# CloudEngineHub/dexrobot_isaac

Measured on AMD Instinct MI355X. Metric: env-steps/sec BlindGrasping num_envs=4096 per MI355X (random actions), higher is better.
Workload: dtype f32

## Files before the change

### dexrobot_isaac_amd/build.py

```python
import os
import shutil
import subprocess

HERE = os.path.dirname(os.path.abspath(__file__))
CSRC = os.path.join(HERE, "csrc")
LIB = os.path.join(HERE, "libdexsim.so")
SOURCES = ["dexsim.hip", "dexsim_device.h", "dexsim_physics.hip.inc", "dexsim_l2.hip.inc"]


DEBUG_SPIN_LIB = os.path.join(HERE, "libdexsim_dbgspin.so")


def _stale(lib=LIB):
    if not os.path.exists(lib):
        return True
    t = os.path.getmtime(lib)
    deps = [os.path.join(CSRC, s) for s in SOURCES] + [os.path.join(HERE, "..", "include", "dexsim.h")]
    return any(os.path.getmtime(d) > t for d in deps if os.path.exists(d))


def build_debug_spin(force=False, bound=2000000):
    return build_lib(force=force, defs=(f"-DDEXSIM_DEBUG_SPIN={int(bound)}",), out=DEBUG_SPIN_LIB)


def build_lib(force=False, verbose=False, defs=(), out=None):
    lib = out or LIB
    if not force and not _stale(lib):
        return lib
    hipcc = shutil.which("hipcc") or "/opt/rocm/bin/hipcc"
    if not os.path.exists(hipcc):
        raise RuntimeError("hipcc not found: libdexsim.so cannot be built on this machine")
    cmd = [hipcc, "--offload-arch=gfx950", "-O3", "-fno-slp-vectorize", "-fno-hip-fp32-correctly-rounded-divide-sqrt",
           "-mllvm", "-amdgpu-sched-strategy=max-ilp", "-fPIC", "-shared", "-std=c++17", *defs,
           "-o", lib, os.path.join(CSRC, "dexsim.hip")]
    if verbose:
        print(" ".join(cmd))
    subprocess.check_call(cmd, cwd=CSRC)
    return lib


if __name__ == "__main__":
    print(build_lib(force=True, verbose=True))
```

### dexrobot_isaac_amd/csrc/dexsim_device.h

```cpp
#pragma once
#include <hip/hip_runtime.h>

#include "../../include/dexsim.h"

#define DEXSIM_FIELDS(X)                                                                                    \
                                \
  X(float, q, 26) X(float, qd, 26) X(float, targets, 26)                                                    \
  X(float, box_pos, 3) X(float, box_quat, 4) X(float, box_lin, 3) X(float, box_ang, 3)                      \
  X(float, box_mass, 1) X(float, box_mu, 1)                                                                 \
                                                \
  X(float, site_pose, 77) X(float, hand_vel, 6) X(float, cforce, 51) X(float, cf5, 15)                      \
                                                    \
  X(float, jframe, 156) X(float, ufree, 32) X(float, fac_finv, 60)                                          \
  X(float, fac_g, 120) X(int, ncontact, 1) X(float, cgeom, DEXSIM_KMAX * 8) X(int, ccode, DEXSIM_KMAX)      \
  X(float, crow, DEXSIM_KMAX * 3 * 28) X(float, crowq, DEXSIM_KMAX * 3 * 28 + 4) X(float, clam, DEXSIM_KMAX * 3) X(float, chdr, DEXSIM_KMAX * 8) X(float, cstage, 6 * NP_STAGE * 9)                                         \
   \
  X(float, wlam, DEXSIM_NWKEY * 4) X(int, wgen, 1) X(int, csplit, 1)                                         \
        \
  X(float, active_prev_targets, 18) X(float, active_rule_targets, 18) X(float, prev_actions, 18)            \
  X(float, actions, 18) X(float, prev_dof_pos, 26)                                                          \
  X(float, contact_duration_steps, 5) X(float, prev_contact_binary, 5) X(int, episode_step, 1)              \
  X(int, success_duration_steps, 1) X(int, success_conditions_met, 1) X(int, current_stage, 1)              \
  X(int, just2, 1) X(int, just3, 1) X(float, time_in_stage, 1) X(float, stage_contact_duration, 1)          \
  X(float, initial_box_pos, 3)                                                                              \
// ... 33 lines not shown
  float box_inv_I_k;
  float base_A[4][3], base_Oc[4][3], base_Q3z[4];
  unsigned obs_div_magic;
  int inertia_diag;
  float hand_reach;
  int obs_col_row[DEXSIM_OBS_ALL_DIM];
  JC jc[DEXSIM_NJ];
  Arena arena;
};

#define CNT_ANY_RESET 0
#define CNT_SUCC 1
#define CNT_FAIL 2
#define CNT_TERM_SUCCESS 8
#define CNT_TERM_FAILURE 9
#define CNT_TERM_TIMEOUT 10
#define CNT_NUM_RESETS 11
#define CNT_CONTACTS 16
#define CNT_HAND_CONTACTS 18
#define CNT_SPIN_TIMEOUT 20
#define CNT_PHYS_STEPS 13
#define CNT_CONSECUTIVE 14
#define CNT_RC_FIRST 15

typedef float f2 __attribute__((ext_vector_type(2)));
typedef float f4 __attribute__((ext_vector_type(4)));
__device__ __forceinline__ void st4_global(float* p, f4 v) { *(__attribute__((address_space(1))) f4*)p = v; }
__device__ __forceinline__ void st4_global(float* p, float a, float b, float c, float d) { f4 v; v.x = a; v.y = b; v.z = c; v.w = d; st4_global(p, v); }

struct V3 { float x, y, z; };
struct Q4 { float x, y, z, w; };
struct S6 { float xx, yy, zz, xy, xz, yz; };
struct M3 { float m[9]; };

#define DI __device__ __forceinline__

DI V3 v3(float x, float y, float z) { return {x, y, z}; }
DI V3 v3p(const float* p) { return {p[0], p[1], p[2]}; }
DI V3 operator+(V3 a, V3 b) { return {a.x + b.x, a.y + b.y, a.z + b.z}; }
DI V3 operator-(V3 a, V3 b) { return {a.x - b.x, a.y - b.y, a.z - b.z}; }
DI V3 operator*(float s, V3 a) { return {s * a.x, s * a.y, s * a.z}; }
DI V3& operator+=(V3& a, V3 b) { a.x += b.x; a.y += b.y; a.z += b.z; return a; }
DI V3& operator-=(V3& a, V3 b) { a.x -= b.x; a.y -= b.y; a.z -= b.z; return a; }
DI float dot(V3 a, V3 b) { return a.x * b.x + a.y * b.y + a.z * b.z; }
DI V3 cross(V3 a, V3 b) { return {a.y * b.z - a.z * b.y, a.z * b.x - a.x * b.z, a.x * b.y - a.y * b.x}; }
DI float norm(V3 a) { return sqrtf(dot(a, a)); }
// ... 171 lines not shown
```

### dexrobot_isaac_amd/csrc/dexsim_l2.hip.inc

```

struct CouplingGroup { int n, dof[3]; float scale[3]; };
constexpr CouplingGroup kCoupling[18] = {
    {1, {0}, {1}}, {1, {1}, {1}}, {1, {2}, {1}}, {1, {3}, {1}}, {1, {4}, {1}}, {1, {5}, {1}},
    {1, {6}, {1}},
    {1, {7}, {1}},
    {2, {8, 9}, {1, 1}},
    {3, {10, 18, 22}, {1, 1, 2}},
    {1, {11}, {1}}, {2, {12, 13}, {1, 1}},
    {1, {15}, {1}}, {2, {16, 17}, {1, 1}},
    {1, {19}, {1}}, {2, {20, 21}, {1, 1}},
    {1, {23}, {1}}, {2, {24, 25}, {1, 1}},
};
constexpr int kHeldDof = 14;
constexpr int kActiveFingerDof[12] = {8, 7, 6, 10, 12, 11, 16, 15, 20, 19, 24, 23};

enum {
#define X(name, dim) O_##name, O_##name##_last = O_##name + (dim) - 1,
  DEXSIM_OBS_KEYS(X)
#undef X
  O_end
};
static_assert(O_end == DEXSIM_OBS_ALL_DIM, "DEXSIM_OBS_ALL_DIM is not the sum of the DEXSIM_OBS_KEYS dims");
static_assert(O_object_pos == DEXSIM_OBS_BASE_TASK_DIM, "DEXSIM_OBS_BASE_TASK_DIM is not the row of object_pos");

DI void begin_step_counters(int* cnt, int stamp) {
  const int o = (stamp & 1) ^ 1;
  cnt[CNT_CONTACTS + o] = 0; cnt[CNT_HAND_CONTACTS + o] = 0;
}

DI void actions_block(const Arena& A, const ApiPtrs& T, const DevParams* __restrict__ P, const float* __restrict__ act,
                      int zero_targets, int N, int NR) {
  const int wv = threadIdx.x >> 6, lane = threadIdx.x & 63;
  const int e = blockIdx.x * 64 + lane;
  const DexSimConfig& C = P->cfg;
  const int na = C.num_actions;
  const bool real = e < NR;
  if (blockIdx.x == 0 && threadIdx.x == 0) begin_step_counters(T.counters, T.stamp);
  const int fs = C.policy_controls_base ? 6 : 0;
  if (wv == 0) {
    FLD(targets, kHeldDof) = 0.f;
    if (real && T.full_dof_targets) T.full_dof_targets[(size_t)e * 26 + kHeldDof] = 0.f;
  }
#pragma unroll
  for (int i = 0; i < 18; i++) {
    if (i / 3 != wv) continue;
    const float ai = (real && i < na) ? act[(size_t)e * na + i] : 0.f;
    const int ci = i < 6 ? i : fs + (i - 6);
    const bool driven = i < 6 ? (C.policy_controls_base != 0) : (C.policy_controls_fingers != 0);
    const float ac = (driven && real && ci < na) ? act[(size_t)e * na + ci] : 0.f;
    float raw = FLD(active_rule_targets, i);
    const float prev = FLD(active_prev_targets, i);
    FLD(actions, i) = ai;
    if (T.actions_copy && real && i < na) T.actions_copy[(size_t)e * na + i] = ai;
    if (T.raw_targets && !zero_targets) {
      raw = real ? T.raw_targets[(size_t)e * 18 + i] : raw;
    } else if (C.control_mode == DEXSIM_MODE_POSITION_DELTA) {
      if (driven) raw = prev + ac * C.max_deltas[i];
      raw = clampf(raw, C.active_lower[i], C.active_upper[i]);
    } else {
      if (driven) raw = (ac + 1.0f) * 0.5f * (C.active_upper[i] - C.active_lower[i]) + C.active_lower[i];
    }
    const float d = clampf(raw - prev, -C.max_deltas[i], C.max_deltas[i]);
    const float nxt = clampf(prev + d, C.active_lower[i], C.active_upper[i]);
    if (!zero_targets) FLD(active_prev_targets, i) = nxt;
    const float tgt = zero_targets ? 0.f : nxt;
    const CouplingGroup& g = kCoupling[i];
#define PUT(k) do { const float t = tgt * g.scale[k]; FLD(targets, g.dof[k]) = t; \
                    if (real && T.full_dof_targets) T.full_dof_targets[(size_t)e * 26 + g.dof[k]] = t; } while (0)
    PUT(0);
    if (g.n > 1) PUT(1);
    if (g.n > 2) PUT(2);
#undef PUT
    FLD(prev_actions, i) = ai;
  }
}

__global__ __launch_bounds__(384) void k_actions(Arena A, ApiPtrs T, const DevParams* __restrict__ P, const float* __restrict__ act,
                                                 int zero_targets, int N, int NR) {
  actions_block(P->arena, T, P, act, zero_targets, N, NR);
}

DI V3 site_pos(const Arena& A, int N, int e, int s) { return {FLD(site_pose, 7 * s), FLD(site_pose, 7 * s + 1), FLD(site_pose, 7 * s + 2)}; }
DI Q4 site_quat(const Arena& A, int N, int e, int s) {
  return {FLD(site_pose, 7 * s + 3), FLD(site_pose, 7 * s + 4), FLD(site_pose, 7 * s + 5), FLD(site_pose, 7 * s + 6)};
}
#define OB_STRIDE (DEXSIM_OBS_ALL_DIM + 1)
#define OB(i) s_ob[lane * OB_STRIDE + (i)]

#ifdef DEXSIM_PROFILE_PHASES
#define PB_STAMP(k) do { if (threadIdx.x == 0) A.crow[(size_t)(32 + (k)) * N + blockIdx.x * 64] = __int_as_float((int)(__builtin_amdgcn_s_memtime() - pb_t0)); } while (0)
#else
#define PB_STAMP(k) do {} while (0)
#endif
#define ST_PEN 0
#define ST_FV2 1
#define ST_FA2 2
#define ST_RC 3
#define ST_WORDS (ST_RC + DEXSIM_NUM_REWROWS + 1)
#define ST(i) s_st[(i) * 64 + lane]
#define POST_NTASK 12

DI void post_task(int t, const Arena& A, const DevParams* __restrict__ P, const int* __restrict__ cnt, float* s_ob, float* s_st,
// ... 540 lines not shown
    for (int g = wv; g < (DEXSIM_NUM_REWROWS + 1 + 3) / 4; g += nw) {
      const int row = 4 * g + r4;
      if (row <= DEXSIM_NUM_REWROWS) {
        const float* sr = s_st + (ST_RC + row) * 64 + 4 * l16;
        const f4 v = {sr[0], sr[1], sr[2], sr[3]};
        float* dst = row < DEXSIM_NUM_REWROWS ? A.rew_comp + (size_t)row * N : A.rew;
        st4_global(dst + blockIdx.x * 64 + 4 * l16, v);
      }
    }
  }
  POST_STAMP();
  POST_STAMP();
#undef POST_STAMP
}

#define POST_LDS_BYTES ((64 * OB_STRIDE + 64 * ST_WORDS + DEXSIM_OBS_ALL_DIM) * sizeof(float))
__global__ __launch_bounds__(512) void k_post(Arena A, ApiPtrs T, const DevParams* __restrict__ P, int* __restrict__ cnt,
                                              int obs_only, int fold_reset, int N, int NR) {
  extern __shared__ float s_post[];
  post_block(P->arena, T, P, cnt, s_post, obs_only, fold_reset, N, NR, 0);
}

DI void finalize_stats(const ApiPtrs& T, const DevParams* __restrict__ P, int NR) {
  int* cnt = T.counters;
  float* st = T.stats;
  const DexSimConfig& C = P->cfg;
  auto mean = [&](int count) { return (float)((double)count / (double)NR); };
  st[DEXSIM_STAT_SUCC_MEAN] = mean(cnt[CNT_SUCC]);
  for (int i = 0; i < DEXSIM_NUM_FAIL; i++) st[DEXSIM_STAT_FAIL_MEAN + i] = mean(cnt[CNT_FAIL + i]);
  st[DEXSIM_STAT_SUCCESS_RATE] = mean(cnt[CNT_TERM_SUCCESS]);
  st[DEXSIM_STAT_FAILURE_RATE] = mean(cnt[CNT_TERM_FAILURE]);
  st[DEXSIM_STAT_TIMEOUT_RATE] = mean(cnt[CNT_TERM_TIMEOUT]);
  int cs = cnt[CNT_TERM_SUCCESS] > 0 ? cnt[CNT_CONSECUTIVE] + 1 : 0;
  if (cs > C.max_consecutive_successes) cs = C.max_consecutive_successes;
  cnt[CNT_CONSECUTIVE] = cs;
  st[DEXSIM_STAT_CONSECUTIVE_SUCCESSES] = (float)cs;
  st[DEXSIM_STAT_NUM_RESETS] = (float)cnt[CNT_NUM_RESETS];
  st[DEXSIM_STAT_PHYSICS_STEPS] = cnt[CNT_ANY_RESET] == T.stamp ? 2.f : 1.f;
  st[DEXSIM_STAT_MEAN_CONTACTS] = mean(cnt[CNT_CONTACTS + (T.stamp & 1)]);
  st[DEXSIM_STAT_MEAN_HAND_CONTACTS] = mean(cnt[CNT_HAND_CONTACTS + (T.stamp & 1)]);
  cnt[CNT_RC_FIRST] = 0;
  for (int i = CNT_SUCC; i <= CNT_NUM_RESETS; i++) cnt[i] = 0;
  if (T.sink_stats)
    for (int i = 0; i < DEXSIM_STAT_USED; i++) T.sink_stats[i] = st[i];
}

DI void reset_phase1(const Arena& A, int N, int e) {
#pragma unroll
  for (int f = 0; f < 5; f++) { FLD(contact_duration_steps, f) = 0.f; FLD(prev_contact_binary, f) = 0.f; }
#pragma unroll
  for (int i = 0; i < 26; i++) FLD(prev_dof_pos, i) = 0.f;
#pragma unroll
  for (int i = 0; i < 18; i++) FLD(prev_actions, i) = 0.f;
}

DI void reset_phase0(const Arena& A, const ApiPtrs& T, const DevParams* __restrict__ P, int N, int NR, int e) {
  const DexSimConfig& C = P->cfg;
  FLD(episode_success, 0) = 0; FLD(episode_failure, 0) = 0; FLD(success_reason, 0) = 0;
#pragma unroll
  for (int i = 0; i < DEXSIM_NUM_FAIL; i++) FLD(failure_reason, i) = 0;
  FLD(episode_step, 0) = 0;
  T.episode_step_count[e] = 0;
  T.episode_length[e] = 0;
  if (T.masks) {
#pragma unroll
    for (int i = 0; i < DEXSIM_NUM_SUCC + DEXSIM_NUM_FAIL; i++) T.masks[(size_t)(DEXSIM_MASK_SUCC_REASON + i) * NR + e] = 0;
  }
// ... 41 lines not shown
  }
#pragma unroll
  for (int c = 0; c < 18; c++) {
    const CouplingGroup& g = kCoupling[c];
    FLD(active_prev_targets, c) = q[g.dof[g.n - 1]] / g.scale[g.n - 1];
  }
}

__global__ __launch_bounds__(64) void k_reset(Arena A, ApiPtrs T, const DevParams* __restrict__ P, const int64_t* __restrict__ ids, int k,
                                              int mode, int phase, int N, int NR) {
  int e = blockIdx.x * 64 + threadIdx.x;
  if (mode == 3) {
    if (e >= NR || FLD(reset_flag, 0) == 0) return;
  } else {
    if (e >= k) return;
    if (mode == 1) e = (int)ids[e];
    if (e < 0 || e >= NR) return;
  }
  if (phase == 1) reset_phase1(A, N, e);
  else reset_phase0(A, T, P, N, NR, e);
}

__global__ void k_finalize(ApiPtrs T, const DevParams* __restrict__ P, int NR) {
  if (threadIdx.x != 0 || blockIdx.x != 0) return;
  finalize_stats(T, P, NR);
}

__global__ void k_begin_step(int* cnt, int stamp) {
  if (threadIdx.x == 0 && blockIdx.x == 0) begin_step_counters(cnt, stamp);
}

__global__ __launch_bounds__(64) void k_init(Arena A, ApiPtrs T, const DevParams* __restrict__ P, int N, int NR) {
  const int e = blockIdx.x * 64 + threadIdx.x;
  const DexSimConfig& C = P->cfg;
  FLD(box_quat, 3) = 1.f;
  FLD(box_pos, 2) = C.box_z;
  FLD(initial_box_pos, 2) = C.box_z;
  if (C.box_fixed) {
#pragma unroll
    for (int i = 0; i < 3; i++) { FLD(box_pos, i) = C.box_fixed_pos[i]; FLD(initial_box_pos, i) = C.box_fixed_pos[i]; }
  }
  float mass = C.box_mass > 0.f ? C.box_mass : 1.f, mu = C.box_friction;
  if (C.dr_enabled) {
    uint32_t x[4];
    philox4x32(x, (uint32_t)e, 0u, 0u, 0u, C.dr_seed, 0xd12au);
    mass = C.dr_mass_lo + u01(x[0]) * (C.dr_mass_hi - C.dr_mass_lo);
    mu = C.dr_mu_lo + u01(x[1]) * (C.dr_mu_hi - C.dr_mu_lo);
// ... 24 lines not shown
```

### dexrobot_isaac_amd/csrc/dexsim_physics.hip.inc

```

#define GPTR(p) ((__attribute__((address_space(1))) __typeof__(*(p))*)(p))
#define FLD(f, r) GPTR(A.f)[(size_t)(r) * N + e]
#define ROWADDR(w, lane) ((((w) >> 2) * 64 + (lane)) * 4 + ((w) & 3))

DI int wave_role(int w) { return w == 2 ? 5 : ((w >= 3 && w <= 5) ? w - 1 : w); }
#ifndef SPEC_SPLIT_NUM
#define SPEC_SPLIT_NUM 12
#endif

#define CODE_TYPE(c) ((c) & 3)
#define CODE_CAP(c) (((c) >> 2) & 31)
#define CODE_SAMPLE(c) (((c) >> 7) & 7)
#define CODE_FINGER(c) ((((c) >> 16) & 7) - 1)
#define CODE_LEVEL(c) (((c) >> 19) & 3)
#define CODE_FSLOT(c) (((c) >> 21) & 31)
DI int code_info(const DexHandModel& M, int cap) {
  const int jp = M.cap_parent[cap];
  return ((jp >= 6 ? ((jp - 6) >> 2) + 1 : 0) << 16) | ((jp >= 6 ? (jp - 6) & 3 : 0) << 19) | (M.cap_fslot[cap] << 21);
}
#define CODE_HKEY(c) (CODE_TYPE(c) == 3 ? 88 + ((CODE_FINGER(c) * 4 + CODE_LEVEL(c)) * 2 + (CODE_SAMPLE(c) & 1)) \
                                         : (CODE_CAP(c) * 2 + CODE_TYPE(c)) * 2 + (CODE_SAMPLE(c) & 1))
#define SPLIT_NB(s) ((s) & 15)
#define SPLIT_NX(s) (((s) >> 4) & 15)
#define SPLIT_NF(s, f) (((s) >> (8 + 4 * (f))) & 15)
// ... 232 lines not shown
    const float reach = (0.5f * norm(d) + r + co) * 1.0001f + 1e-6f;
    clear = clear && !(dot(ex, ex) < reach * reach);
  }
  return clear;
}

#define SH(i) sh[(i) * 64 + lane]
DI void sh_put3(float* sh, int lane, int i, V3 v) { SH(i) = v.x; SH(i + 1) = v.y; SH(i + 2) = v.z; }
DI void comp_put(float* sh, int lane, int w, const Comp& c, V3 o5) {
  const V3 d = c.c - o5;
  const S6 J = c.I + pa(c.m, d);
  sh[(w) * 64 + lane] = c.m; sh_put3(sh, lane, w + 1, d);
  sh[(w + 4) * 64 + lane] = J.xx; sh[(w + 5) * 64 + lane] = J.yy; sh[(w + 6) * 64 + lane] = J.zz;
  sh[(w + 7) * 64 + lane] = J.xy; sh[(w + 8) * 64 + lane] = J.xz; sh[(w + 9) * 64 + lane] = J.yz;
}
DI V3 sh_get3(const float* sh, int lane, int i) { return {SH(i), SH(i + 1), SH(i + 2)}; }
DI void bch_get2(const float* s_bch, int lane, int i2, V3& a0, V3& o0, V3& a1, V3& o1) {
  const f4 q0 = *(const f4*)(s_bch + ROWADDR(12 * i2, lane)), q1 = *(const f4*)(s_bch + ROWADDR(12 * i2 + 4, lane)),
           q2 = *(const f4*)(s_bch + ROWADDR(12 * i2 + 8, lane));
  a0 = {q0.x, q0.y, q0.z}; o0 = {q0.w, q1.x, q1.y}; a1 = {q1.z, q1.w, q2.x}; o1 = {q2.y, q2.z, q2.w};
}


#define DL_SINV 0
#define DL_SCHUR_S 0
#define DL_SCHUR_GSUM 27
#define DL_PALM 36
#define DL_PALM_WRENCH 46
#define DL_NC 52
#define DL_PERSIST 53
#define DL_SSUB(b, f) ((b) + (f) * 43)
#define DL_GSUM(b, f) ((b) + (f) * 43 + 21)
#define DL_COMP(b, f) ((b) + (f) * 43 + 27)
#define DL_WRENCH(b, f) ((b) + (f) * 43 + 37)
#define DL_CAPS(b, f) ((b) + 215 + (f) * 18)
#define DL_HANDOFF 305
#define DL_WORDS (DL_PERSIST + DL_HANDOFF)
#define DL_SPLIT DL_WORDS

#define FS_UB 53
#define FS_BOXV 59
#define FS_UF 65
#define FS_LAM 85
#define FS_HDR 157
#define FS_ROW 197
#define FS_HDR_HI 197
// ... 9 lines not shown
#define FS_CARRY_QD 606
#define FS_CARRY_BP 612
#define FS_COMPCNT 615
#define FS_GEN 617
#define FS_SPLIT 618
#define FS_CPACK 619
#define FS_CMP_INVM 620
#define FS_FLAG 622
#define FS_CARRY_Q 628
#define FS_TGTB 634
#define FS_WORDS 640
#define FS_LDS_BYTES (FS_WORDS * 64 * sizeof(float))

enum : unsigned { LIVE_ACROSS = 1u << 6, LIVE_PUB = 1u << 7, LIVE_POST = 1u << 8 };
constexpr unsigned lds_live(int first, int last) {
  unsigned m = 0;
  for (int p = first; p <= last; p++) m |= 1u << (p == 0 ? 1 : p);
  return m;
}
constexpr unsigned LIVE_CARRY = lds_live(5, 5) | LIVE_ACROSS | lds_live(0, 0);
constexpr unsigned LIVE_LAUNCH = lds_live(0, 5) | LIVE_ACROSS;
struct LdsRegion { int start, words; unsigned live; };
constexpr LdsRegion LDS_MAP[] = {
  {DL_SINV,      36,                      lds_live(2, 3)},
  {DL_PALM,      16,                      lds_live(1, 2)},
  {DL_NC,        1,                       lds_live(1, 5)},
  {FS_UB,        6,                       lds_live(2, 5)},
  {FS_BOXV,      6,                       lds_live(1, 5)},
  {FS_UF,        20,                      lds_live(1, 5)},
  {FS_LAM,       3 * DEXSIM_KMAX,         lds_live(1, 5)},
  {FS_HDR,       FS_HDR_HI - FS_HDR,      lds_live(1, 5)},
  {FS_ROW,       DL_HANDOFF,              lds_live(1, 2)},
  {FS_HDR_HI,    4 * DEXSIM_KMAX - (FS_HDR_HI - FS_HDR), lds_live(3, 5)},
  {FS_X,         13 * 5 * 4,              lds_live(3, 4)},
  {FS_FORCE,     5 * 3 * DEXSIM_NFSLOT,   lds_live(5, 5)},
  {FS_T,         8 * 4,                   lds_live(3, 4)},
  {FS_SPRE,      27,                      lds_live(1, 2)},
  {FS_BCH,       36,                      lds_live(1, 3)},
  {FS_CTAB,      12,                      lds_live(2, 4)},
  {FS_NITEM,     1,                       lds_live(2, 4)},
  {FS_CMP,       12,                      lds_live(1, 4)},
  {FS_CARRY_QD,  6,                       LIVE_CARRY},
  {FS_CARRY_BP,  3,                       LIVE_CARRY},
  {FS_COMPCNT,   1,                       LIVE_LAUNCH},
  {FS_GEN,       1,                       lds_live(1, 4)},
  {FS_SPLIT,     1,                       lds_live(2, 4)},
// ... 1640 lines not shown
      }
      if (wv < 5) {
        const f4 t = *TQ(3 + wv);
        s_uf[(4 * wv) * 64 + lane] = t.x; s_uf[(4 * wv + 1) * 64 + lane] = t.y; s_uf[(4 * wv + 2) * 64 + lane] = t.z;
        s_uf[(4 * wv + 3) * 64 + lane] = t.w;
      } else {
        const f4 t0 = *TQ(0), t1 = *TQ(1);
        SH(FS_UB) = t0.x; SH(FS_UB + 1) = t0.y; SH(FS_UB + 2) = t0.z; SH(FS_UB + 3) = t0.w; SH(FS_UB + 4) = t1.x; SH(FS_UB + 5) = t1.y;
        SH(FS_BOXV) = t1.z; SH(FS_BOXV + 1) = t1.w;
      }
    }
  }
  GP_STAMP(4);
  if (wv == 6) __builtin_amdgcn_s_setprio(2);
  __syncthreads();
  if (probe && wv == 0 && lane == 0) atomicAdd(probe + blockIdx.x * 4 + 3, (unsigned)(__builtin_amdgcn_s_memtime() - pr_t4));
}
#undef GP_STAMP
#undef SWEEP_STAMP

struct SubstepCarry { float ql[4], qdl[4], tg[4]; };
template <bool LAST>
DI void substep_body(const Arena& A, const ApiPtrs& T, const DevParams* __restrict__ P, int* __restrict__ cnt, int N, int NR, float* sh,
                     int seq, int stamp_base, bool post_pre, bool count_contacts, SubstepCarry& carry, bool carry_in, bool carry_out) {
  constexpr int dlb = FS_ROW;
  int* const ccnt = count_contacts ? cnt + (T.stamp & 1) : nullptr;
  constexpr int last = LAST ? 1 : 0;
  const int wv = __builtin_amdgcn_readfirstlane(wave_role(threadIdx.x >> 6)), lane = threadIdx.x & 63;
  const int e = blockIdx.x * 64 + lane;
#ifdef DEXSIM_PROFILE_PHASES
  const unsigned long long t_start = __builtin_amdgcn_s_memtime();
  int stamp_i = 0;
#ifdef DBG_PH2
#define PH2_STAMP(i) do { if (lane == 0 && (wv == 1 || wv == 5)) A.crow[(size_t)(stamp_base + 56 + (i) + (wv == 5 ? 4 : 0)) * N + e] = __int_as_float((int)(__builtin_amdgcn_s_memtime() - t_start)); } while (0)
#else
#define PH2_STAMP(i) do {} while (0)
#endif
#define PHASE_STAMP() do { if (lane == 0) A.crow[(size_t)(stamp_base + wv * 8 + stamp_i) * N + e] = __int_as_float((int)(__builtin_amdgcn_s_memtime() - t_start)); stamp_i++; } while (0)
#else
#define PH2_STAMP(i) do {} while (0)
#define PHASE_STAMP() do {} while (0)
#endif
  {
  const DexHandModel& M = P->model;
  const DexSimConfig& C = P->cfg;
  const float h = P->h;
  const V3 grav = v3p(C.gravity);
  const bool has_box = C.has_box != 0;
  float* s_uf = sh + FS_UF * 64;
  float* s_lam = sh + FS_LAM * 64;
  float* s_hdr = sh + FS_HDR * 64;
  if (wv == 6) __builtin_amdgcn_s_setprio(2);
  BaseChain B;
  FingerIn fin;
  bool hand_free = false, sphere = false;
  V3 bpos_h = {0, 0, 0};
  M3 Rb_h = q2mat(Q4{0, 0, 0, 1});
  if (wv != 6) {
    if (carry_in) {
      if (has_box) bpos_h = {SH(FS_CARRY_BP), SH(FS_CARRY_BP + 1), SH(FS_CARRY_BP + 2)};
      base_chain(A, P, grav, N, e, B, false, sh + FS_CARRY_Q * 64, sh + FS_CARRY_QD * 64, lane);
      if (wv < 5) {
#pragma unroll
        for (int l = 0; l < 4; l++) { fin.ql[l] = carry.ql[l]; fin.qdl[l] = carry.qdl[l]; fin.tg[l] = carry.tg[l]; }
      }
    } else {
      if (has_box) bpos_h = {FLD(box_pos, 0), FLD(box_pos, 1), FLD(box_pos, 2)};
      base_chain(A, P, grav, N, e, B, false);
      if (wv < 5) finger_load(A, wv, N, e, fin);
    }
    sphere = hand_clear(P, B, bpos_h);
    if (!sphere && has_box) Rb_h = q2mat(Q4{FLD(box_quat, 0), FLD(box_quat, 1), FLD(box_quat, 2), FLD(box_quat, 3)});
    if (wv == 5) {
      bool pclear = sphere;
      if (!sphere) {
        const M3 R5 = q2mat(B.q5);
        bool clr = true;
#pragma unroll
        for (int cpl = 0; cpl < 3; cpl++)
          clr = clr && capsule_clear(B.o5 + mul(R5, v3p(M.cap_p0[cpl])), B.o5 + mul(R5, v3p(M.cap_p1[cpl])), M.cap_r[cpl], C, bpos_h, Rb_h);
        pclear = __all(clr);
      }
      if (lane == 0) sh[(FS_FLAG + 5) * 64] = __int_as_float((seq << 1) | (pclear ? 1 : 0));
    }
  }
  PHASE_STAMP();

  int nc = 0, nbg = 0;
  float Gkeep[24];
#pragma unroll
  for (int i = 0; i < 24; i++) Gkeep[i] = 0.f;
  V3 bpos = {0, 0, 0}; M3 Rb = q2mat(Q4{0, 0, 0, 1});
  float hb = 0.f, bmu = 0.f;
  if (wv < 5) {
    finger_dynamics(A, P, B, fin, sh, dlb, s_uf, lane, wv, N, e, seq, sphere, bpos_h, Rb_h, Gkeep);
  } else if (wv == 5) {
    const M3 R5 = q2mat(B.q5);
    Comp comp5;
    comp5.m = P->jc[5].mass;
    comp5.c = B.o5 + mul(R5, v3p(P->jc[5].com));
    comp5.I = rotate_inertia(R5, P->jc[5].inertia);
    V3 rc = comp5.c - B.o5;
    V3 ac = B.ao5 + cross(B.al5, rc) + cross(B.w5, cross(B.w5, rc));
    V3 f5 = comp5.m * ac;
    V3 n5 = mul(comp5.I, B.al5) + cross(B.w5, mul(comp5.I, B.w5)) + cross(rc, f5);
    comp_put(sh, lane, DL_PALM, comp5, B.o5);
    sh_put3(sh, lane, DL_PALM_WRENCH, f5); sh_put3(sh, lane, DL_PALM_WRENCH + 3, n5);
#pragma unroll
    for (int i = 0; i < 6; i++) SH(FS_TGTB + i) = FLD(targets, i);
#pragma unroll
    for (int i2 = 0; i2 < 3; i2++) {
      const V3 a0 = B.ab[2 * i2], o0 = B.ob[2 * i2], a1 = B.ab[2 * i2 + 1], o1 = B.ob[2 * i2 + 1];
      *(f4*)(sh + FS_BCH * 64 + ROWADDR(12 * i2, lane)) = f4{a0.x, a0.y, a0.z, o0.x};
      *(f4*)(sh + FS_BCH * 64 + ROWADDR(12 * i2 + 4, lane)) = f4{o0.y, o0.z, a1.x, a1.y};
      *(f4*)(sh + FS_BCH * 64 + ROWADDR(12 * i2 + 8, lane)) = f4{a1.z, o1.x, o1.y, o1.z};
    }
    schur_precompute(sh, dlb, lane, B, seq, cnt);
  } else if (wv == 6) {
    float bv[6] = {0, 0, 0, 0, 0, 0};
    const int gen = FLD(wgen, 0);
    f4 wq[4];
#pragma unroll
    for (int k = 0; k < 4; k++) wq[k] = *(const __attribute__((address_space(1))) f4*)(A.wlam + ((size_t)(80 + k) * N + e) * 4);
    int cpack = 0;
    SH(FS_GEN) = __int_as_float(gen);
    if (has_box) {
      bpos = {FLD(box_pos, 0), FLD(box_pos, 1), FLD(box_pos, 2)};
      Rb = q2mat(Q4{FLD(box_quat, 0), FLD(box_quat, 1), FLD(box_quat, 2), FLD(box_quat, 3)});
      hb = 0.5f * C.box_size;
      bmu = FLD(box_mu, 0);
      const float mu_bg = 0.5f * (bmu + C.ground_friction);
      const bool bfix = C.box_fixed != 0;
// ... 336 lines not shown
      if (carry_out) { SH(FS_CARRY_BP) = fmaf(h, vb[0], bpos.x); SH(FS_CARRY_BP + 1) = fmaf(h, vb[1], bpos.y); SH(FS_CARRY_BP + 2) = fmaf(h, vb[2], bpos.z); }
      if (!C.box_fixed) integrate_box(A, h, vb, wb, N, e);
    }
  }
  if (last && wv < 5 && gp) forces_reduce(A, ccnt, s_hdr, sh + FS_FORCE * 64, nc, lane, N, e, NR, wv, 5);
  if (last && wv == 5 && gp) contact_stats(ccnt, s_hdr, nc, lane, e, NR);
  PHASE_STAMP();
  }
  if (LAST) {
    __syncthreads();
    publish_body(A, T, P, 0, N, NR, 6);
    if (post_pre && wv == 6) post_pre_tasks(A, P, cnt, sh, N);
    PHASE_STAMP();
  }
#undef PHASE_STAMP
#undef PH2_STAMP
}

DI void reset_phase1(const Arena& A, int N, int e);
DI void finalize_stats(const ApiPtrs& T, const DevParams* __restrict__ P, int NR);
DI void post_block(const Arena& A, const ApiPtrs& T, const DevParams* __restrict__ P, int* __restrict__ cnt, float* s_ob,
                   int obs_only, int fold_reset, int N, int NR, int done_mask);
DI void actions_block(const Arena& A, const ApiPtrs& T, const DevParams* __restrict__ P, const float* __restrict__ act,
                      int zero_targets, int N, int NR);

enum {
  TAIL_RESET = 1,
  TAIL_POST = 2,
  TAIL_NOT_FINAL = 4,
};

template <bool GATED>
DI unsigned long long physics_prologue(const ApiPtrs& T, float* sh) {
  unsigned long long pr_k0 = 0;
  if (T.probe && threadIdx.x == 0) pr_k0 = __builtin_amdgcn_s_memtime();
  if (threadIdx.x < 6) sh[(FS_FLAG + threadIdx.x) * 64] = 0.f;
  if (threadIdx.x == 6) sh[FS_COMPCNT * 64] = 0.f;
  return pr_k0;
}
template <bool GATED>
DI void physics_epilogue(const ApiPtrs& T, const DevParams* __restrict__ P, int tail, unsigned long long pr_k0, int NR) {
  if (GATED && (tail & TAIL_RESET) && blockIdx.x == 0 && threadIdx.x == 0) finalize_stats(T, P, NR);
  if (!GATED && T.probe && threadIdx.x == 0) atomicAdd(T.probe + blockIdx.x * 4 + 1, (unsigned)(__builtin_amdgcn_s_memtime() - pr_k0));
}

template <bool GATED>
__global__ __launch_bounds__(448) void k_physics4(Arena A, ApiPtrs T, const DevParams* __restrict__ P, int* __restrict__ cnt,
                                                  const float* __restrict__ act, int tail, int N, int NR) {
  extern __shared__ float sh[];
  const unsigned long long pr_k0 = physics_prologue<GATED>(T, sh);
  if (!GATED && act) actions_block(P->arena, T, P, act, 0, N, NR);
  __syncthreads();
  if (!GATED || cnt[CNT_ANY_RESET] == T.stamp) {
    SubstepCarry K;
    substep_body<false>(P->arena, T, P, cnt, N, NR, sh, 1, 64, false, true, K, false, true);
    __syncthreads();
    substep_body<false>(P->arena, T, P, cnt, N, NR, sh, 2, 128, false, true, K, true, true);
    __syncthreads();
    substep_body<false>(P->arena, T, P, cnt, N, NR, sh, 3, 192, false, true, K, true, true);
    __syncthreads();
    substep_body<true>(P->arena, T, P, cnt, N, NR, sh, 4, 256, !GATED && (tail & TAIL_POST), !GATED && !(tail & TAIL_NOT_FINAL), K, true, false);
    if (!GATED && (tail & TAIL_POST)) {
      __syncthreads();
      post_block(P->arena, T, P, cnt, sh, 0, 1, N, NR, POST_PRE_MASK);
    }
    if (GATED && (tail & TAIL_RESET)) {
      const int e = blockIdx.x * 64 + (threadIdx.x & 63);
      if (threadIdx.x < 64 && e < NR && A.reset_flag[e] != 0) reset_phase1(A, N, e);
    }
  }
  physics_epilogue<GATED>(T, P, tail, pr_k0, NR);
}

template <bool GATED>
__global__ __launch_bounds__(448) void k_physics1(Arena A, ApiPtrs T, const DevParams* __restrict__ P, int* __restrict__ cnt,
                                                  const float* __restrict__ act, int tail, int N, int NR) {
  extern __shared__ float sh[];
  const unsigned long long pr_k0 = physics_prologue<GATED>(T, sh);
  if (!GATED && act) actions_block(P->arena, T, P, act, 0, N, NR);
  __syncthreads();
  if (!GATED || cnt[CNT_ANY_RESET] == T.stamp) {
    SubstepCarry K;
    substep_body<true>(P->arena, T, P, cnt, N, NR, sh, 1, 0, !GATED && (tail & TAIL_POST), !GATED && !(tail & TAIL_NOT_FINAL), K, false, false);
    if (!GATED && (tail & TAIL_POST)) {
      __syncthreads();
      post_block(P->arena, T, P, cnt, sh, 0, 1, N, NR, POST_PRE_MASK);
    }
    if (GATED && (tail & TAIL_RESET)) {
      const int e = blockIdx.x * 64 + (threadIdx.x & 63);
      if (threadIdx.x < 64 && e < NR && A.reset_flag[e] != 0) reset_phase1(A, N, e);
    }
  }
  physics_epilogue<GATED>(T, P, tail, pr_k0, NR);
}
```

Measured before the change: 65.91 million.

## Stage first-substep state and action targets through LDS, early-exit gated physics

New measurement: 65.91 million (median of 2 runs). About the same (+0.0%).

```diff
diff --git a/dexrobot_isaac_amd/build.py b/dexrobot_isaac_amd/build.py
--- a/dexrobot_isaac_amd/build.py
+++ b/dexrobot_isaac_amd/build.py
@@ -9,6 +9,8 @@
 
 
 DEBUG_SPIN_LIB = os.path.join(HERE, "libdexsim_dbgspin.so")
+FLAGS = ["--offload-arch=gfx950", "-O3", "-fno-slp-vectorize", "-fno-hip-fp32-correctly-rounded-divide-sqrt",
+         "-mllvm", "-amdgpu-sched-strategy=max-ilp", "-std=c++17"]
 
 
 def _stale(lib=LIB):
@@ -30,9 +32,7 @@
     hipcc = shutil.which("hipcc") or "/opt/rocm/bin/hipcc"
     if not os.path.exists(hipcc):
         raise RuntimeError("hipcc not found: libdexsim.so cannot be built on this machine")
-    cmd = [hipcc, "--offload-arch=gfx950", "-O3", "-fno-slp-vectorize", "-fno-hip-fp32-correctly-rounded-divide-sqrt",
-           "-mllvm", "-amdgpu-sched-strategy=max-ilp", "-fPIC", "-shared", "-std=c++17", *defs,
-           "-o", lib, os.path.join(CSRC, "dexsim.hip")]
+    cmd = [hipcc, *FLAGS, "-fPIC", "-shared", *defs, "-o", lib, os.path.join(CSRC, "dexsim.hip")]
     if verbose:
         print(" ".join(cmd))
     subprocess.check_call(cmd, cwd=CSRC)
diff --git a/dexrobot_isaac_amd/csrc/dexsim_device.h b/dexrobot_isaac_amd/csrc/dexsim_device.h
--- a/dexrobot_isaac_amd/csrc/dexsim_device.h
+++ b/dexrobot_isaac_amd/csrc/dexsim_device.h
@@ -79,6 +79,10 @@
 #define CNT_PHYS_STEPS 13
 #define CNT_CONSECUTIVE 14
 #define CNT_RC_FIRST 15
+#define CNT_FINALIZE_WORDS 32
+static_assert(CNT_HAND_CONTACTS + 2 <= CNT_FINALIZE_WORDS && CNT_RC_FIRST < CNT_FINALIZE_WORDS && CNT_FINALIZE_WORDS <= DEXSIM_STAT_WORDS,
+              "counters block: a word of the step statistics lies outside finalize_stats' one load");
+static_assert(CNT_SPIN_TIMEOUT >= CNT_HAND_CONTACTS + 2, "counters block: the diagnostic word overlaps the contact statistics");
 
 typedef float f2 __attribute__((ext_vector_type(2)));
 typedef float f4 __attribute__((ext_vector_type(4)));
diff --git a/dexrobot_isaac_amd/csrc/dexsim_l2.hip.inc b/dexrobot_isaac_amd/csrc/dexsim_l2.hip.inc
--- a/dexrobot_isaac_amd/csrc/dexsim_l2.hip.inc
+++ b/dexrobot_isaac_amd/csrc/dexsim_l2.hip.inc
@@ -28,56 +28,90 @@
   cnt[CNT_CONTACTS + o] = 0; cnt[CNT_HAND_CONTACTS + o] = 0;
 }
 
-DI void actions_block(const Arena& A, const ApiPtrs& T, const DevParams* __restrict__ P, const float* __restrict__ act,
-                      int zero_targets, int N, int NR) {
-  const int wv = threadIdx.x >> 6, lane = threadIdx.x & 63;
+template <int W>
+DI void actions_wave(const Arena& A, const ApiPtrs& T, const DevParams* __restrict__ P, const float* __restrict__ act,
+                     int zero_targets, int N, int NR, float* s_tgt) {
+  const int lane = threadIdx.x & 63;
   const int e = blockIdx.x * 64 + lane;
   const DexSimConfig& C = P->cfg;
   const int na = C.num_actions;
   const bool real = e < NR;
-  if (blockIdx.x == 0 && threadIdx.x == 0) begin_step_counters(T.counters, T.stamp);
   const int fs = C.policy_controls_base ? 6 : 0;
-  if (wv == 0) {
+  const bool host_raw = T.raw_targets && !zero_targets;
+  float ai[3], ac[3], raw[3], prev[3], hraw[3], maxd[3], lo[3], hi[3];
+  bool driven[3];
+#pragma unroll
+  for (int k = 0; k < 3; k++) {
+    constexpr int i0 = 3 * W;
+    const int i = i0 + k;
+    ai[k] = (real && i < na) ? act[(size_t)e * na + i] : 0.f;
+    const int ci = i < 6 ? i : fs + (i - 6);
+    driven[k] = i < 6 ? (C.policy_controls_base != 0) : (C.policy_controls_fingers != 0);
+    ac[k] = (driven[k] && real && ci < na) ? act[(size_t)e * na + ci] : 0.f;
+    raw[k] = FLD(active_rule_targets, i);
+    prev[k] = FLD(active_prev_targets, i);
+    hraw[k] = (host_raw && real) ? T.raw_targets[(size_t)e * 18 + i] : 0.f;
+    maxd[k] = C.max_deltas[i]; lo[k] = C.active_lower[i]; hi[k] = C.active_upper[i];
+  }
+  const int mode = C.control_mode;
+#pragma unroll
+  for (int k = 0; k < 3; k++) asm volatile("" ::"s"(maxd[k]), "s"(lo[k]), "s"(hi[k]), "s"(mode));
+  float nxt[3], tgt[3];
+#pragma unroll
+  for (int k = 0; k < 3; k++) {
+    float r = raw[k];
+    if (host_raw) {
+      r = real ? hraw[k] : r;
+    } else if (mode == DEXSIM_MODE_POSITION_DELTA) {
+      if (driven[k]) r = prev[k] + ac[k] * maxd[k];
+      r = clampf(r, lo[k], hi[k]);
+    } else {
+      if (driven[k]) r = (ac[k] + 1.0f) * 0.5f * (hi[k] - lo[k]) + lo[k];
+    }
+    const float d = clampf(r - prev[k], -maxd[k], maxd[k]);
+    nxt[k] = clampf(prev[k] + d, lo[k], hi[k]);
+    tgt[k] = zero_targets ? 0.f : nxt[k];
+  }
+  if (W == 0 && blockIdx.x == 0 && lane == 0) begin_step_counters(T.counters, T.stamp);
+  if (W == 0) {
     FLD(targets, kHeldDof) = 0.f;
+    if (s_tgt) s_tgt[kHeldDof * 64 + lane] = 0.f;
     if (real && T.full_dof_targets) T.full_dof_targets[(size_t)e * 26 + kHeldDof] = 0.f;
   }
 #pragma unroll
-  for (int i = 0; i < 18; i++) {
-    if (i / 3 != wv) continue;
-    const float ai = (real && i < na) ? act[(size_t)e * na + i] : 0.f;
-    const int ci = i < 6 ? i : fs + (i - 6);
-    const bool driven = i < 6 ? (C.policy_controls_base != 0) : (C.policy_controls_fingers != 0);
-    const float ac = (driven && real && ci < na) ? act[(size_t)e * na + ci] : 0.f;
-    float raw = FLD(active_rule_targets, i);
-    const float prev = FLD(active_prev_targets, i);
-    FLD(actions, i) = ai;
-    if (T.actions_copy && real && i < na) T.actions_copy[(size_t)e * na + i] = ai;
-    if (T.raw_targets && !zero_targets) {
-      raw = real ? T.raw_targets[(size_t)e * 18 + i] : raw;
-    } else if (C.control_mode == DEXSIM_MODE_POSITION_DELTA) {
-      if (driven) raw = prev + ac * C.max_deltas[i];
-      raw = clampf(raw, C.active_lower[i], C.active_upper[i]);
-    } else {
-      if (driven) raw = (ac + 1.0f) * 0.5f * (C.active_upper[i] - C.active_lower[i]) + C.active_lower[i];
-    }
-    const float d = clampf(raw - prev, -C.max_deltas[i], C.max_deltas[i]);
-    const float nxt = clampf(prev + d, C.active_lower[i], C.active_upper[i]);
-    if (!zero_targets) FLD(active_prev_targets, i) = nxt;
-    const float tgt = zero_targets ? 0.f : nxt;
+  for (int k = 0; k < 3; k++) {
+    constexpr int i0 = 3 * W;
+    const int i = i0 + k;
+    FLD(actions, i) = ai[k];
+    if (T.actions_copy && real && i < na) T.actions_copy[(size_t)e * na + i] = ai[k];
+    if (!zero_targets) FLD(active_prev_targets, i) = nxt[k];
     const CouplingGroup& g = kCoupling[i];
-#define PUT(k) do { const float t = tgt * g.scale[k]; FLD(targets, g.dof[k]) = t; \
-                    if (real && T.full_dof_targets) T.full_dof_targets[(size_t)e * 26 + g.dof[k]] = t; } while (0)
+#define PUT(s) do { const float t = tgt[k] * g.scale[s]; FLD(targets, g.dof[s]) = t; if (s_tgt) s_tgt[g.dof[s] * 64 + lane] = t; \
+                    if (real && T.full_dof_targets) T.full_dof_targets[(size_t)e * 26 + g.dof[s]] = t; } while (0)
     PUT(0);
     if (g.n > 1) PUT(1);
     if (g.n > 2) PUT(2);
 #undef PUT
-    FLD(prev_actions, i) = ai;
+    FLD(prev_actions, i) = ai[k];
+  }
+}
+
+DI void actions_block(const Arena& A, const ApiPtrs& T, const DevParams* __restrict__ P, const float* __restrict__ act,
+                      int zero_targets, int N, int NR, float* s_tgt) {
+  switch (threadIdx.x >> 6) {
+    case 0: actions_wave<0>(A, T, P, act, zero_targets, N, NR, s_tgt); break;
+    case 1: actions_wave<1>(A, T, P, act, zero_targets, N, NR, s_tgt); break;
+    case 2: actions_wave<2>(A, T, P, act, zero_targets, N, NR, s_tgt); break;
+    case 3: actions_wave<3>(A, T, P, act, zero_targets, N, NR, s_tgt); break;
+    case 4: actions_wave<4>(A, T, P, act, zero_targets, N, NR, s_tgt); break;
+    case 5: actions_wave<5>(A, T, P, act, zero_targets, N, NR, s_tgt); break;
+    default: break;
   }
 }
 
 __global__ __launch_bounds__(384) void k_actions(Arena A, ApiPtrs T, const DevParams* __restrict__ P, const float* __restrict__ act,
                                                  int zero_targets, int N, int NR) {
-  actions_block(P->arena, T, P, act, zero_targets, N, NR);
+  actions_block(P->arena, T, P, act, zero_targets, N, NR, nullptr);
 }
 
 DI V3 site_pos(const Arena& A, int N, int e, int s) { return {FLD(site_pose, 7 * s), FLD(site_pose, 7 * s + 1), FLD(site_pose, 7 * s + 2)}; }
@@ -664,27 +698,40 @@
 }
 
 DI void finalize_stats(const ApiPtrs& T, const DevParams* __restrict__ P, int NR) {
+  static_assert(DEXSIM_NUM_SUCC == 1 && CNT_FINALIZE_WORDS <= 64 && DEXSIM_STAT_USED <= 64, "finalize_stats: lane maps");
+  const int lane = threadIdx.x & 63;
   int* cnt = T.counters;
   float* st = T.stats;
   const DexSimConfig& C = P->cfg;
+  const int cw = lane < CNT_FINALIZE_WORDS ? GPTR(cnt)[lane] : 0;
+  float sv = lane < DEXSIM_STAT_USED ? GPTR(st)[lane] : 0.f;
+  const int par = T.stamp & 1;
+  const int max_cs = C.max_consecutive_successes;
+  asm volatile("" ::"s"(max_cs));
   auto mean = [&](int count) { return (float)((double)count / (double)NR); };
-  st[DEXSIM_STAT_SUCC_MEAN] = mean(cnt[CNT_SUCC]);
-  for (int i = 0; i < DEXSIM_NUM_FAIL; i++) st[DEXSIM_STAT_FAIL_MEAN + i] = mean(cnt[CNT_FAIL + i]);
-  st[DEXSIM_STAT_SUCCESS_RATE] = mean(cnt[CNT_TERM_SUCCESS]);
-  st[DEXSIM_STAT_FAILURE_RATE] = mean(cnt[CNT_TERM_FAILURE]);
-  st[DEXSIM_STAT_TIMEOUT_RATE] = mean(cnt[CNT_TERM_TIMEOUT]);
-  int cs = cnt[CNT_TERM_SUCCESS] > 0 ? cnt[CNT_CONSECUTIVE] + 1 : 0;
-  if (cs > C.max_consecutive_successes) cs = C.max_consecutive_successes;
-  cnt[CNT_CONSECUTIVE] = cs;
-  st[DEXSIM_STAT_CONSECUTIVE_SUCCESSES] = (float)cs;
-  st[DEXSIM_STAT_NUM_RESETS] = (float)cnt[CNT_NUM_RESETS];
-  st[DEXSIM_STAT_PHYSICS_STEPS] = cnt[CNT_ANY_RESET] == T.stamp ? 2.f : 1.f;
-  st[DEXSIM_STAT_MEAN_CONTACTS] = mean(cnt[CNT_CONTACTS + (T.stamp & 1)]);
-  st[DEXSIM_STAT_MEAN_HAND_CONTACTS] = mean(cnt[CNT_HAND_CONTACTS + (T.stamp & 1)]);
-  cnt[CNT_RC_FIRST] = 0;
-  for (int i = CNT_SUCC; i <= CNT_NUM_RESETS; i++) cnt[i] = 0;
-  if (T.sink_stats)
-    for (int i = 0; i < DEXSIM_STAT_USED; i++) T.sink_stats[i] = st[i];
+  auto word = [&](int i) { return __builtin_amdgcn_readlane(cw, i); };
+  int count = -1;
+  if (lane == DEXSIM_STAT_SUCC_MEAN) count = word(CNT_SUCC);
+#pragma unroll
+  for (int i = 0; i < DEXSIM_NUM_FAIL; i++)
+    if (lane == DEXSIM_STAT_FAIL_MEAN + i) count = word(CNT_FAIL + i);
+  if (lane == DEXSIM_STAT_SUCCESS_RATE) count = word(CNT_TERM_SUCCESS);
+  if (lane == DEXSIM_STAT_FAILURE_RATE) count = word(CNT_TERM_FAILURE);
+  if (lane == DEXSIM_STAT_TIMEOUT_RATE) count = word(CNT_TERM_TIMEOUT);
+  if (lane == DEXSIM_STAT_MEAN_CONTACTS) count = word(CNT_CONTACTS + par);
+  if (lane == DEXSIM_STAT_MEAN_HAND_CONTACTS) count = word(CNT_HAND_CONTACTS + par);
+  if (count >= 0) sv = mean(count);
+  int cs = word(CNT_TERM_SUCCESS) > 0 ? word(CNT_CONSECUTIVE) + 1 : 0;
+  if (cs > max_cs) cs = max_cs;
+  if (lane == DEXSIM_STAT_CONSECUTIVE_SUCCESSES) sv = (float)cs;
+  if (lane == DEXSIM_STAT_NUM_RESETS) sv = (float)word(CNT_NUM_RESETS);
+  if (lane == DEXSIM_STAT_PHYSICS_STEPS) sv = word(CNT_ANY_RESET) == T.stamp ? 2.f : 1.f;
+  if (lane < DEXSIM_STAT_USED) {
+    GPTR(st)[lane] = sv;
+    if (T.sink_stats) GPTR(T.sink_stats)[lane] = sv;
+  }
+  if (lane == CNT_RC_FIRST || (lane >= CNT_SUCC && lane <= CNT_NUM_RESETS)) GPTR(cnt)[lane] = 0;
+  if (lane == CNT_CONSECUTIVE) GPTR(cnt)[lane] = cs;
 }
 
 DI void reset_phase1(const Arena& A, int N, int e) {
@@ -772,7 +819,7 @@
 }
 
 __global__ void k_finalize(ApiPtrs T, const DevParams* __restrict__ P, int NR) {
-  if (threadIdx.x != 0 || blockIdx.x != 0) return;
+  if (threadIdx.x >= 64 || blockIdx.x != 0) return;
   finalize_stats(T, P, NR);
 }
 
diff --git a/dexrobot_isaac_amd/csrc/dexsim_physics.hip.inc b/dexrobot_isaac_amd/csrc/dexsim_physics.hip.inc
--- a/dexrobot_isaac_amd/csrc/dexsim_physics.hip.inc
+++ b/dexrobot_isaac_amd/csrc/dexsim_physics.hip.inc
@@ -278,6 +278,7 @@
 }
 
 
+#define FS_TGT 0
 #define DL_SINV 0
 #define DL_SCHUR_S 0
 #define DL_SCHUR_GSUM 27
@@ -333,6 +334,7 @@
 constexpr unsigned LIVE_LAUNCH = lds_live(0, 5) | LIVE_ACROSS;
 struct LdsRegion { int start, words; unsigned live; };
 constexpr LdsRegion LDS_MAP[] = {
+  {FS_TGT,       26,                      LIVE_ACROSS | lds_live(0, 1)},
   {DL_SINV,      36,                      lds_live(2, 3)},
   {DL_PALM,      16,                      lds_live(1, 2)},
   {DL_NC,        1,                       lds_live(1, 5)},
@@ -2019,7 +2021,7 @@
 struct SubstepCarry { float ql[4], qdl[4], tg[4]; };
 template <bool LAST>
 DI void substep_body(const Arena& A, const ApiPtrs& T, const DevParams* __restrict__ P, int* __restrict__ cnt, int N, int NR, float* sh,
-                     int seq, int stamp_base, bool post_pre, bool count_contacts, SubstepCarry& carry, bool carry_in, bool carry_out) {
+                     int seq, int stamp_base, bool post_pre, bool count_contacts, SubstepCarry& carry, bool carry_out) {
   constexpr int dlb = FS_ROW;
   int* const ccnt = count_contacts ? cnt + (T.stamp & 1) : nullptr;
   constexpr int last = LAST ? 1 : 0;
@@ -2054,17 +2056,11 @@
   V3 bpos_h = {0, 0, 0};
   M3 Rb_h = q2mat(Q4{0, 0, 0, 1});
   if (wv != 6) {
-    if (carry_in) {
-      if (has_box) bpos_h = {SH(FS_CARRY_BP), SH(FS_CARRY_BP + 1), SH(FS_CARRY_BP + 2)};
-      base_chain(A, P, grav, N, e, B, false, sh + FS_CARRY_Q * 64, sh + FS_CARRY_QD * 64, lane);
-      if (wv < 5) {
-#pragma unroll
-        for (int l = 0; l < 4; l++) { fin.ql[l] = carry.ql[l]; fin.qdl[l] = carry.qdl[l]; fin.tg[l] = carry.tg[l]; }
-      }
-    } else {
-      if (has_box) bpos_h = {FLD(box_pos, 0), FLD(box_pos, 1), FLD(box_pos, 2)};
-      base_chain(A, P, grav, N, e, B, false);
-      if (wv < 5) finger_load(A, wv, N, e, fin);
+    if (has_box) bpos_h = {SH(FS_CARRY_BP), SH(FS_CARRY_BP + 1), SH(FS_CARRY_BP + 2)};
+    base_chain(A, P, grav, N, e, B, false, sh + FS_CARRY_Q * 64, sh + FS_CARRY_QD * 64, lane);
+    if (wv < 5) {
+#pragma unroll
+      for (int l = 0; l < 4; l++) { fin.ql[l] = carry.ql[l]; fin.qdl[l] = carry.qdl[l]; fin.tg[l] = carry.tg[l]; }
     }
     sphere = hand_clear(P, B, bpos_h);
     if (!sphere && has_box) Rb_h = q2mat(Q4{FLD(box_quat, 0), FLD(box_quat, 1), FLD(box_quat, 2), FLD(box_quat, 3)});
@@ -2104,7 +2100,7 @@
     comp_put(sh, lane, DL_PALM, comp5, B.o5);
     sh_put3(sh, lane, DL_PALM_WRENCH, f5); sh_put3(sh, lane, DL_PALM_WRENCH + 3, n5);
 #pragma unroll
-    for (int i = 0; i < 6; i++) SH(FS_TGTB + i) = FLD(targets, i);
+    for (int i = 0; i < 6; i++) SH(FS_TGTB + i) = seq == 1 ? SH(FS_TGT + i) : FLD(targets, i);
 #pragma unroll
     for (int i2 = 0; i2 < 3; i2++) {
       const V3 a0 = B.ab[2 * i2], o0 = B.ob[2 * i2], a1 = B.ab[2 * i2 + 1], o1 = B.ob[2 * i2 + 1];
@@ -2487,13 +2483,67 @@
 DI void post_block(const Arena& A, const ApiPtrs& T, const DevParams* __restrict__ P, int* __restrict__ cnt, float* s_ob,
                    int obs_only, int fold_reset, int N, int NR, int done_mask);
 DI void actions_block(const Arena& A, const ApiPtrs& T, const DevParams* __restrict__ P, const float* __restrict__ act,
-                      int zero_targets, int N, int NR);
+                      int zero_targets, int N, int NR, float* s_tgt);
 
 enum {
   TAIL_RESET = 1,
   TAIL_POST = 2,
   TAIL_NOT_FINAL = 4,
 };
+
+#ifdef DEXSIM_PROFILE_PHASES
+#define KSTAMP_ROW 336
+#define K_STAMP_T0() const unsigned long long k_t0 = __builtin_amdgcn_s_memtime()
+#define K_STAMP(k) do { if ((threadIdx.x & 63) == 0) GPTR(A.crow)[(size_t)(KSTAMP_ROW + 8 * (k) + (threadIdx.x >> 6)) * N + blockIdx.x * 64] = __int_as_float((int)(__builtin_amdgcn_s_memtime() - k_t0)); } while (0)
+#define G_STAMP(k) do { if (GATED && blockIdx.x == 0 && threadIdx.x == 0) { __builtin_amdgcn_s_waitcnt(0); GPTR(A.crow)[(size_t)(KSTAMP_ROW + 16 + (k)) * N] = __int_as_float((int)(__builtin_amdgcn_s_memtime() - k_t0)); } } while (0)
+#else
+#define K_STAMP_T0() do {} while (0)
+#define K_STAMP(k) do {} while (0)
+#define G_STAMP(k) do {} while (0)
+#endif
+
+struct Body0In { float q[6], qd[6], tg[6], bp[3]; };
+DI void body0_load(const Arena& A, const DevParams* __restrict__ P, SubstepCarry& K, Body0In& in, int N) {
+  const int wv = __builtin_amdgcn_readfirstlane(wave_role(threadIdx.x >> 6)), lane = threadIdx.x & 63;
+  const int e = blockIdx.x * 64 + lane;
+#pragma unroll
+  for (int i = 0; i < 6; i++) { in.q[i] = 0.f; in.qd[i] = 0.f; in.tg[i] = 0.f; }
+#pragma unroll
+  for (int i = 0; i < 3; i++) in.bp[i] = 0.f;
+#pragma unroll
+  for (int l = 0; l < 4; l++) { K.ql[l] = 0.f; K.qdl[l] = 0.f; K.tg[l] = 0.f; }
+  if (wv < 5) {
+#pragma unroll
+    for (int l = 0; l < 4; l++) { const int j = 6 + 4 * wv + l; K.ql[l] = FLD(q, j); K.qdl[l] = FLD(qd, j); K.tg[l] = FLD(targets, j); }
+  } else if (wv == 5) {
+#pragma unroll
+    for (int i = 0; i < 6; i++) { in.q[i] = FLD(q, i); in.qd[i] = FLD(qd, i); in.tg[i] = FLD(targets, i); }
+  } else if (P->cfg.has_box) {
+#pragma unroll
+    for (int i = 0; i < 3; i++) in.bp[i] = FLD(box_pos, i);
+  }
+}
+DI void body0_stage(const DevParams* __restrict__ P, bool stage_targets, const Body0In& in, float* sh) {
+  const int wv = __builtin_amdgcn_readfirstlane(wave_role(threadIdx.x >> 6)), lane = threadIdx.x & 63;
+  if (wv == 5) {
+#pragma unroll
+    for (int i = 0; i < 6; i++) { SH(FS_CARRY_Q + i) = in.q[i]; SH(FS_CARRY_QD + i) = in.qd[i]; }
+    if (stage_targets) {
+#pragma unroll
+      for (int i = 0; i < 6; i++) SH(FS_TGT + i) = in.tg[i];
+    }
+  } else if (wv == 6 && P->cfg.has_box) {
+#pragma unroll
+    for (int i = 0; i < 3; i++) SH(FS_CARRY_BP + i) = in.bp[i];
+  }
+}
+DI void body0_targets(bool from_lds, SubstepCarry& K, const float* sh) {
+  const int wv = __builtin_amdgcn_readfirstlane(wave_role(threadIdx.x >> 6)), lane = threadIdx.x & 63;
+  if (from_lds && wv < 5) {
+#pragma unroll
+    for (int l = 0; l < 4; l++) K.tg[l] = SH(FS_TGT + 6 + 4 * wv + l);
+  }
+}
 
 template <bool GATED>
 DI unsigned long long physics_prologue(const ApiPtrs& T, float* sh) {
@@ -2505,7 +2555,7 @@
 }
 template <bool GATED>
 DI void physics_epilogue(const ApiPtrs& T, const DevParams* __restrict__ P, int tail, unsigned long long pr_k0, int NR) {
-  if (GATED && (tail & TAIL_RESET) && blockIdx.x == 0 && threadIdx.x == 0) finalize_stats(T, P, NR);
+  if (GATED && (tail & TAIL_RESET) && blockIdx.x == 0 && threadIdx.x < 64) finalize_stats(T, P, NR);
   if (!GATED && T.probe && threadIdx.x == 0) atomicAdd(T.probe + blockIdx.x * 4 + 1, (unsigned)(__builtin_amdgcn_s_memtime() - pr_k0));
 }
 
@@ -2513,18 +2563,35 @@
 __global__ __launch_bounds__(448) void k_physics4(Arena A, ApiPtrs T, const DevParams* __restrict__ P, int* __restrict__ cnt,
                                                   const float* __restrict__ act, int tail, int N, int NR) {
   extern __shared__ float sh[];
+  K_STAMP_T0();
+  if (GATED) {
+    const bool gate_open = cnt[CNT_ANY_RESET] == T.stamp;
+    G_STAMP(0);
+    if (!gate_open) {
+      physics_epilogue<GATED>(T, P, tail, 0, NR);
+      G_STAMP(1);
+      return;
+    }
+  }
   const unsigned long long pr_k0 = physics_prologue<GATED>(T, sh);
-  if (!GATED && act) actions_block(P->arena, T, P, act, 0, N, NR);
+  const bool with_act = !GATED && act;
+  SubstepCarry K;
+  Body0In in0;
+  body0_load(P->arena, P, K, in0, N);
+  if (with_act) actions_block(P->arena, T, P, act, 0, N, NR, sh + FS_TGT * 64);
+  body0_stage(P, !with_act, in0, sh);
+  K_STAMP(0);
   __syncthreads();
-  if (!GATED || cnt[CNT_ANY_RESET] == T.stamp) {
-    SubstepCarry K;
-    substep_body<false>(P->arena, T, P, cnt, N, NR, sh, 1, 64, false, true, K, false, true);
+  {
+    K_STAMP(1);
+    body0_targets(with_act, K, sh);
+    substep_body<false>(P->arena, T, P, cnt, N, NR, sh, 1, 64, false, true, K, true);
     __syncthreads();
-    substep_body<false>(P->arena, T, P, cnt, N, NR, sh, 2, 128, false, true, K, true, true);
+    substep_body<false>(P->arena, T, P, cnt, N, NR, sh, 2, 128, false, true, K, true);
     __syncthreads();
-    substep_body<false>(P->arena, T, P, cnt, N, NR, sh, 3, 192, false, true, K, true, true);
+    substep_body<false>(P->arena, T, P, cnt, N, NR, sh, 3, 192, false, true, K, true);
     __syncthreads();
-    substep_body<true>(P->arena, T, P, cnt, N, NR, sh, 4, 256, !GATED && (tail & TAIL_POST), !GATED && !(tail & TAIL_NOT_FINAL), K, true, false);
+    substep_body<true>(P->arena, T, P, cnt, N, NR, sh, 4, 256, !GATED && (tail & TAIL_POST), !GATED && !(tail & TAIL_NOT_FINAL), K, false);
     if (!GATED && (tail & TAIL_POST)) {
       __syncthreads();
       post_block(P->arena, T, P, cnt, sh, 0, 1, N, NR, POST_PRE_MASK);
@@ -2535,18 +2602,36 @@
     }
   }
   physics_epilogue<GATED>(T, P, tail, pr_k0, NR);
+  G_STAMP(1);
 }
 
 template <bool GATED>
 __global__ __launch_bounds__(448) void k_physics1(Arena A, ApiPtrs T, const DevParams* __restrict__ P, int* __restrict__ cnt,
                                                   const float* __restrict__ act, int tail, int N, int NR) {
   extern __shared__ float sh[];
+  K_STAMP_T0();
+  if (GATED) {
+    const bool gate_open = cnt[CNT_ANY_RESET] == T.stamp;
+    G_STAMP(0);
+    if (!gate_open) {
+      physics_epilogue<GATED>(T, P, tail, 0, NR);
+      G_STAMP(1);
+      return;
+    }
+  }
   const unsigned long long pr_k0 = physics_prologue<GATED>(T, sh);
-  if (!GATED && act) actions_block(P->arena, T, P, act, 0, N, NR);
+  const bool with_act = !GATED && act;
+  SubstepCarry K;
+  Body0In in0;
+  body0_load(P->arena, P, K, in0, N);
+  if (with_act) actions_block(P->arena, T, P, act, 0, N, NR, sh + FS_TGT * 64);
+  body0_stage(P, !with_act, in0, sh);
+  K_STAMP(0);
   __syncthreads();
-  if (!GATED || cnt[CNT_ANY_RESET] == T.stamp) {
-    SubstepCarry K;
-    substep_body<true>(P->arena, T, P, cnt, N, NR, sh, 1, 0, !GATED && (tail & TAIL_POST), !GATED && !(tail & TAIL_NOT_FINAL), K, false, false);
+  {
+    K_STAMP(1);
+    body0_targets(with_act, K, sh);
+    substep_body<true>(P->arena, T, P, cnt, N, NR, sh, 1, 0, !GATED && (tail & TAIL_POST), !GATED && !(tail & TAIL_NOT_FINAL), K, false);
     if (!GATED && (tail & TAIL_POST)) {
       __syncthreads();
       post_block(P->arena, T, P, cnt, sh, 0, 1, N, NR, POST_PRE_MASK);
@@ -2557,4 +2642,5 @@
     }
   }
   physics_epilogue<GATED>(T, P, tail, pr_k0, NR);
-}
+  G_STAMP(1);
+}
```
